# noirmist/Pytorch_Pose_Proposal_Network

Hardware: AMD Instinct MI355X
Metric: images/sec (384x384, DRN-D-22) at 1/2/4/8 MI355X (higher is better)
Workload: dtype bf16

## Files before the change

include/ppn.h:

```cpp
#ifndef PPN_H
#define PPN_H

#include <stddef.h>
#include <stdint.h>

#ifdef __cplusplus
extern "C" {
#endif

#define PPN_OK 0
#define PPN_E_INVALID (-1)
#define PPN_E_HIP (-2)
#define PPN_E_UNSUPPORTED (-3)

#define PPN_MAX_EDGES 32
#define PPN_MAX_KP 32

const char* ppn_last_error(void);
int ppn_version(void);

typedef struct ppn_decode_cfg {
    int32_t K, E;
    int32_t sH, sW;
    int32_t H, W;
// ... 113 lines not shown
#define PPN_CONV_NO_FILTER_BANK 1
#define PPN_CONV_SHARED_GPU 2
#define PPN_CONV_OUT_BF16 4
#define PPN_CONV_X3_PLAIN_OUT 8

int ppn_conv_tiling(int32_t dtype, int32_t cin, int32_t cout, int32_t ksize, int32_t* k_step, int32_t* cout_tile,
                    int32_t* k_order);

int ppn_conv2d_fused(const ppn_conv_desc* d, void* stream);

typedef struct ppn_block_desc {
    int32_t dtype;
    int32_t batch, h, w, channels;
    const void* src;
    const void* residual;
    const void* weight1;
    const float* scale_mid;
    const float* shift_mid;
    int32_t act_mid;
    const void* weight2;
    const float* scale1;
    const float* shift1;
    int32_t act1;
    const float* scale2;
    const float* shift2;
    int32_t act2;
    void* out_raw;
    void* out_act;
    int32_t flags;
    int32_t stride, in_h, in_w;
    const void* proj_src;
    const void* proj_weight;
    const float* proj_scale;
    const float* proj_shift;
    int32_t w1_ld, proj_ld;
} ppn_block_desc;
int ppn_basicblock64_fused(const ppn_block_desc* d, void* stream);

int ppn_pack_weight_x3(const float* w, int32_t cout, int32_t cin, int32_t ksize, int32_t cout_pad, int32_t scale_log2,
                       void* out, void* stream);
int ppn_split_f16x3(const float* src, int64_t pixels, int32_t channels, void* dst, void* stream);

int ppn_conv_split(int32_t dtype, int32_t cin, int32_t cout, int64_t m, int64_t* m_split);

int ppn_ingest_frames(const void* src_bgr, int32_t batch, int32_t src_h, int32_t src_w, void* dst_rgb, int32_t dst_h,
                      int32_t dst_w, int32_t flip, int32_t swap_rb, void* stream);

int ppn_set_conv_tile_policy(int32_t policy);

int ppn_set_conv_tile_override(int32_t bp, int32_t bc);

int ppn_set_conv64_enabled(int32_t on);

const char* ppn_last_conv_kernel(void);

int ppn_stem7x7(int32_t dtype, int32_t src_is_u8, const void* src, int32_t batch, int32_t h, int32_t w,
                const float* weight, const float* scale, const float* shift, const float* mean, const float* std_,
                void* out, void* stream);

int ppn_stem01(int32_t dtype, int32_t src_is_u8, const void* src, int32_t batch, int32_t h, int32_t w,
               const float* w0, const float* scale0, const float* shift0, const float* mean, const float* std_,
               const float* w1, const float* scale1, const float* shift1, void* out, void* stream);

typedef struct ppn_plan ppn_plan;
int ppn_plan_create(ppn_plan** out);
int ppn_plan_add_conv(ppn_plan* p, const ppn_conv_desc* d);
int ppn_plan_add_block(ppn_plan* p, const ppn_block_desc* d);
int ppn_plan_add_memset(ppn_plan* p, void* ptr, size_t bytes);
int ppn_plan_add_split(ppn_plan* p, const float* src, int64_t pixels, int32_t channels, void* dst);
int ppn_plan_add_stem(ppn_plan* p, int32_t dtype, int32_t src_is_u8, const void* src, int32_t batch, int32_t h,
                      int32_t w, const float* weight, const float* scale, const float* shift, const float* mean,
                      const float* std_, void* out);
int ppn_plan_add_stem01(ppn_plan* p, int32_t dtype, int32_t src_is_u8, const void* src, int32_t batch, int32_t h,
                        int32_t w, const float* w0, const float* scale0, const float* shift0, const float* mean,
                        const float* std_, const float* w1, const float* scale1, const float* shift1, void* out);
int ppn_stem012(int32_t src_is_u8, const void* src, int32_t batch, int32_t h, int32_t w, const float* w0,
                const float* scale0, const float* shift0, const float* mean, const float* std_, const float* w1,
                const float* scale1, const float* shift1, const float* w2, const float* scale2, const float* shift2,
                const float* scale3, const float* shift3, void* out_raw, void* out_act, void* stream);
int ppn_plan_add_stem012(ppn_plan* p, int32_t src_is_u8, const void* src, int32_t batch, int32_t h, int32_t w,
                         const float* w0, const float* scale0, const float* shift0, const float* mean, const float* std_,
                         const float* w1, const float* scale1, const float* shift1, const float* w2, const float* scale2,
                         const float* shift2, const float* scale3, const float* shift3, void* out_raw, void* out_act);
#define PPN_STEM_IO(internal, out) ((internal) | (((out) + 1) << 8))
#define PPN_STEM_RAW_S2 (1 << 16)
int ppn_stem012_dt(int32_t dtype, int32_t src_is_u8, const void* src, int32_t batch, int32_t h, int32_t w, const float* w0,
                   const float* scale0, const float* shift0, const float* mean, const float* std_, const float* w1,
                   const float* scale1, const float* shift1, const float* w2, const float* scale2, const float* shift2,
                   const float* scale3, const float* shift3, void* out_raw, void* out_act, void* stream);
int ppn_plan_add_stem012_dt(ppn_plan* p, int32_t dtype, int32_t src_is_u8, const void* src, int32_t batch, int32_t h,
                            int32_t w, const float* w0, const float* scale0, const float* shift0, const float* mean,
                            const float* std_, const float* w1, const float* scale1, const float* shift1, const float* w2,
                            const float* scale2, const float* shift2, const float* scale3, const float* shift3,
                            void* out_raw, void* out_act);
int ppn_plan_set_input(ppn_plan* p, const void* src);
int ppn_plan_run(ppn_plan* p, void* stream);
int ppn_plan_run_timed(ppn_plan* p, void* stream, float* ms, int32_t n_ms, int32_t repeats);
int ppn_plan_graph_captures(const ppn_plan* p);
int ppn_plan_size(const ppn_plan* p);
const char* ppn_plan_kernel_name(const ppn_plan* p, int32_t i);
int ppn_plan_destroy(ppn_plan* p);

int ppn_pack_weight(int32_t dtype, const float* w, int32_t cout, int32_t cin, int32_t ksize, int32_t cout_pad,
                    int32_t k_total, int32_t k_order, int32_t k_step, void* out, void* stream);
int ppn_pack_weight_dgrad(int32_t dtype, const float* w, int32_t cout, int32_t cin, int32_t ksize, int32_t cout_pad,
                          int32_t k_total, int32_t k_order, int32_t k_step, void* out, void* stream);
// ... 142 lines not shown
```

pytorch_pose_proposal_network_amd/csrc/conv_big.hip:

```cpp
#include <algorithm>
#include <cstdio>
#include <cstdlib>
#include <type_traits>
#include <utility>

#include "conv_common.h"

namespace {

using namespace ppnconv;

constexpr bool stats_tile_ok(int bp, int bc) {
    return bc >= 128 && (size_t)bp * (size_t)(bc * 2 + 16) <= 2 * (size_t)(bp + bc) * 128;
}

#ifndef PPN_DIAG
#define PPN_DIAG 0
#endif
constexpr unsigned kOOB = 0x80000000u;

template <typename F, int... I>
__device__ __forceinline__ void static_for_impl(F&& f, std::integer_sequence<int, I...>) {
    (f(std::integral_constant<int, I>{}), ...);
}
template <int N, typename F>
__device__ __forceinline__ void static_for(F&& f) {
    static_for_impl(f, std::make_integer_sequence<int, N>{});
}

template <typename T>
__device__ __forceinline__ void load4(const char* p, float* v);
template <>
__device__ __forceinline__ void load4<float>(const char* p, float* v) {
    const float4 a = *reinterpret_cast<const float4*>(p);
    v[0] = a.x; v[1] = a.y; v[2] = a.z; v[3] = a.w;
}
template <>
__device__ __forceinline__ void load4<__bf16>(const char* p, float* v) {
    const uint2 a = *reinterpret_cast<const uint2*>(p);
    v[0] = __uint_as_float(a.x << 16); v[1] = __uint_as_float(a.x & 0xffff0000u);
    v[2] = __uint_as_float(a.y << 16); v[3] = __uint_as_float(a.y & 0xffff0000u);
}
template <>
__device__ __forceinline__ void load4<_Float16>(const char* p, float* v) {
    typedef __attribute__((ext_vector_type(4))) _Float16 f16x4;
    const f16x4 a = *reinterpret_cast<const f16x4*>(p);
#pragma unroll
    for (int i = 0; i < 4; ++i) v[i] = (float)a[i];
}
template <typename T>
__device__ __forceinline__ void store4(char* p, const float* v);
template <>
__device__ __forceinline__ void store4<float>(char* p, const float* v) {
    *reinterpret_cast<float4*>(p) = make_float4(v[0], v[1], v[2], v[3]);
}
template <>
__device__ __forceinline__ void store4<__bf16>(char* p, const float* v) {
    typedef __attribute__((ext_vector_type(4))) __bf16 bf16x4;
    bf16x4 o;
#pragma unroll
    for (int i = 0; i < 4; ++i) o[i] = (__bf16)v[i];
    *reinterpret_cast<bf16x4*>(p) = o;
}

template <>
__device__ __forceinline__ void store4<_Float16>(char* p, const float* v) {
    typedef __attribute__((ext_vector_type(4))) _Float16 f16x4;
    f16x4 o;
#pragma unroll
    for (int i = 0; i < 4; ++i) o[i] = (_Float16)clamp_f16(v[i]);
    *reinterpret_cast<f16x4*>(p) = o;
}

__device__ __forceinline__ void bufload_lds16(__amdgpu_buffer_rsrc_t rsrc, char* lds_wave_base, unsigned voff,
                                              unsigned soff) {
    __builtin_amdgcn_raw_ptr_buffer_load_lds(rsrc, (void __attribute__((address_space(3)))*)lds_wave_base, 16, voff,
                                             soff, 0, 0);
}

template <typename T, int BP, int BC, int NW, bool SC, bool X3 = false, bool ST = false>
__global__ void __launch_bounds__(64 * NW, (ST && BP == 192 && BC == 128) ? 4 : NW / 4)
conv_igemm_big_kernel(ConvKArgs a, unsigned src_bytes, unsigned wgt_bytes) {
    static_assert(!X3 || (std::is_same<T, _Float16>::value && !SC), "X3 is the split-f16 mode without a fused shortcut");
    static_assert(!ST || (sizeof(T) == 2 && !SC && !X3 && NW == 8 && BC >= 128), "ST: plain 16-bit launches of the 8-wave tiles");
    constexpr int EPC = Elem<T>::EPC;
    constexpr int BK = 8 * EPC;
    constexpr int ES = sizeof(T);
    constexpr int NT = 64 * NW;
    constexpr int WC = (BP % (16 * (NW / 2)) == 0) ? 2 : NW;
    constexpr int WP = NW / WC;
    constexpr int NXI = (BP + 8 * NW - 1) / (8 * NW), NWI = BC / (8 * NW);
    constexpr bool XRAGGED = BP % (8 * NW) != 0;
    constexpr int TP = BP / WP / 16, TC = BC / WC / 16;
    constexpr int STAGE = (BP + BC) * 128;
    static_assert(BP % 8 == 0 && BC % (8 * NW) == 0 && (BP / WP) % 16 == 0 && BC % (16 * WC) == 0, "tile shape");
    static_assert(TP <= 9 && TC <= 8 && TC * TP % 2 == 0, "accumulators must fit the register file");

    extern __shared__ __attribute__((aligned(16))) char smem[];
#ifdef PPN_CLOCK
    const unsigned long long ck_entry = __builtin_amdgcn_s_memtime();
    const unsigned long long rk_entry = __builtin_amdgcn_s_memrealtime();
#endif
    const int tid = threadIdx.x, lane = tid & 63;
    const int wave = __builtin_amdgcn_readfirstlane(tid >> 6);
    const int wc = wave / WP, wp = wave % WP;

    int ptile, ctile;
    {
        const int nb = gridDim.x, id = blockIdx.x;
        const int xcd = id & 7, loc = id >> 3, q = nb >> 3, r = nb & 7;
        const int logical = (xcd < r ? xcd * (q + 1) : r * (q + 1) + (xcd - r) * q) + loc;
        ptile = fast_div(logical, a.div_nct);
        ctile = logical - ptile * a.n_ctiles;
    }
    const int m0 = a.m_base + ptile * BP, c0 = ctile * BC;

    const __amdgpu_buffer_rsrc_t xrs = __builtin_amdgcn_make_buffer_rsrc((void*)a.src, 0, src_bytes, 0x00020000);
    const __amdgpu_buffer_rsrc_t wrs = __builtin_amdgcn_make_buffer_rsrc((void*)a.wgt, 0, wgt_bytes, 0x00020000);
    const __amdgpu_buffer_rsrc_t xrs2 =
        __builtin_amdgcn_make_buffer_rsrc((void*)(SC ? a.src2 : a.src), 0, SC ? a.src2_bytes : 0u, 0x00020000);

    const int lrow = lane >> 3;
    const int chunk = (lane & 7) ^ (((lane >> 4) & 3) | ((wave & 1) << 2));
    const int ntaps = a.ks * a.ks;
    int xbase[NXI];
    int xbase2[NXI];
    unsigned xmask[NXI];
#pragma unroll
    for (int j = 0; j < NXI; ++j) {
        const int row = (j * NW + wave) * 8 + lrow;
        const int m = m0 + row;
        const bool vm = m < a.M;
        const int mm = vm ? m : 0;
        const int b = fast_div(mm, a.div_howo), rem = mm - b * a.HoWo;
        const int oy = fast_div(rem, a.div_wo), ox = rem - oy * a.Wo;
        const int iy0 = oy * a.stride - a.pad, ix0 = ox * a.stride - a.pad;
        xbase[j] = (((b * a.H + iy0) * a.W + ix0) * a.Cin + chunk * EPC) * ES;
        unsigned mk = 0, cx = 0;
#pragma unroll
        for (int dx = 0; dx < 5; ++dx)
            cx |= (dx < a.ks && (unsigned)(ix0 + dx * a.dil) < (unsigned)a.W) ? (1u << dx) : 0u;
#pragma unroll
        for (int dy = 0; dy < 5; ++dy)
            mk |= (dy < a.ks && (unsigned)(iy0 + dy * a.dil) < (unsigned)a.H) ? (cx << (dy * a.ks)) : 0u;
        mk = vm ? mk : 0u;
        xmask[j] = mk | (vm ? 0x80000000u : 0u);
        if constexpr (SC)
            xbase2[j] = (((b * a.H2 + oy * a.stride2) * a.W2 + ox * a.stride2) * a.Cin2 + chunk * EPC) * ES;
        else
            xbase2[j] = 0;
    }
    unsigned woff[NWI];
#pragma unroll
    for (int j = 0; j < NWI; ++j) {
        const int row = (j * NW + wave) * 8 + lrow;
        woff[j] = (unsigned)(((size_t)(c0 + row) * a.Ktot + chunk * EPC) * ES);
    }

    const int nsteps = a.Ktot / BK;
    const int dx_bytes = a.dil * a.Cin * ES;
    const int dy_bytes = a.dil * a.W * a.Cin * ES - a.ks * dx_bytes;
    const int ksz = a.ks;
    int u_tap = 0, u_dx = 0, u_slab = 0, tapoff = 0, u_ph = 0;
    unsigned tapbit = 1u;
    unsigned ksoff = 0;
    bool live = true;
    bool phase2 = a.nsteps_main == 0;
    int ld_step = 0;
// ... 74 lines not shown
            wf[r - TP] = *reinterpret_cast<const f32x4*>(smem + buf * STAGE + w_tile_off + foff[ks] + (r - TP) * 16 * 128);
    };
    constexpr int GS = (TC * TP % 4 == 0) ? 4 : ((TC * TP % 3 == 0) ? 3 : 2);
    constexpr int NG = TC * TP / GS;
#if PPN_DIAG == 3 || PPN_DIAG == 4
    typedef float f32x16 __attribute__((ext_vector_type(16)));
    f32x16 acc32[TC * TP / 4];
#pragma unroll
    for (int i = 0; i < TC * TP / 4; ++i)
#pragma unroll
        for (int j = 0; j < 16; ++j) acc32[i][j] = 0.f;
#endif
    auto mma_group = [&](auto gc, const f32x4 (&wf)[TC], const f32x4 (&xf)[TP]) {
        constexpr int g = decltype(gc)::value;
#if PPN_DIAG == 3 || PPN_DIAG == 4
        if constexpr (std::is_same<T, __bf16>::value) {
            constexpr int i0 = g * 4, i1 = g * 4 + 3;
            acc32[g] = __builtin_amdgcn_mfma_f32_32x32x16_bf16(__builtin_bit_cast(bf16x8, wf[i0 / TP]),
                                                               __builtin_bit_cast(bf16x8, xf[i0 % TP]), acc32[g], 0, 0, 0);
            acc32[g] = __builtin_amdgcn_mfma_f32_32x32x16_bf16(__builtin_bit_cast(bf16x8, wf[i1 / TP]),
                                                               __builtin_bit_cast(bf16x8, xf[i1 % TP]), acc32[g], 0, 0, 0);
            return;
        }
#endif
        static_for<GS>([&](auto tc) {
            constexpr int idx = g * GS + decltype(tc)::value;
            mma_step(acc[idx / TP][idx % TP], wf[idx / TP], xf[idx % TP], (T*)nullptr);
        });
    };
    constexpr int RPG = (NRD + NG - 1) / NG;
    constexpr int LPG = (NL + NG - 1) / NG;

#ifdef PPN_CLOCK
    const unsigned long long ck_state = __builtin_amdgcn_s_memtime();
#endif
    static_for<NL>([&](auto gc) { issue_one(gc, 0); });
    advance();
    static_for<NL>([&](auto gc) { issue_one(gc, 1); });
    advance();
    if constexpr (XRAGGED) {
        if ((NXI - 1) * NW * 8 + wave * 8 < BP) asm volatile("s_waitcnt vmcnt(%0)" ::"n"(NL) : "memory");
        else asm volatile("s_waitcnt vmcnt(%0)" ::"n"(NL - 1) : "memory");
    } else {
        asm volatile("s_waitcnt vmcnt(%0)" ::"n"(NL) : "memory");
    }
    __syncthreads();
#ifdef PPN_CLOCK
    const unsigned long long ck_bar = __builtin_amdgcn_s_memtime();
#endif
    static_for<NRD>([&](auto rc) { read_one(rc, wA, xA, 0, 0); });
    static_for<NRD>([&](auto rc) { read_one(rc, wB, xB, 0, 1); });
    static_for<NG>([&](auto gc) { mma_group(gc, wA, xA); });
    asm volatile("s_waitcnt vmcnt(0) lgkmcnt(0)" ::: "memory");
    __syncthreads();

#ifdef PPN_STAMP
    unsigned long long st_b1 = 0, st_b2 = 0, st_wait = 0, st_bar = 0, tq0, tq1;
#define PPN_T(var) do { __builtin_amdgcn_sched_barrier(0); asm volatile("s_memtime %0\n\ts_waitcnt lgkmcnt(0)" : "=s"(var) :: "memory"); __builtin_amdgcn_sched_barrier(0); } while (0)
#else
#define PPN_T(var) do { } while (0)
#endif
#ifdef PPN_CLOCK
    const unsigned long long ck0 = __builtin_amdgcn_s_memtime(), rk0 = __builtin_amdgcn_s_memrealtime();
#endif
    for (int s = 1; s < nsteps; ++s) {
        const int buf = s & 1;
#ifdef PPN_STAMP
        PPN_T(tq0);
#endif
        static_for<NG>([&](auto gc) {
            constexpr int g = decltype(gc)::value;
            mma_group(gc, wB, xB);
#if PPN_DIAG != 2 && PPN_DIAG != 4 && PPN_DIAG != 5 && PPN_DIAG != 6
            static_for<LPG>([&](auto lc) {
                constexpr int l = g * LPG + decltype(lc)::value;
                if constexpr (l < NL) issue_one(std::integral_constant<int, l>{}, buf ^ 1);
            });
#endif
            static_for<RPG>([&](auto rc) {
                constexpr int r = g * RPG + decltype(rc)::value;
                if constexpr (r < NRD) read_one(std::integral_constant<int, r>{}, wA, xA, buf, 0);
            });
            __builtin_amdgcn_sched_barrier(0);
        });
        advance();
#ifdef PPN_STAMP
        PPN_T(tq1); st_b1 += tq1 - tq0;
#endif
        static_for<NG>([&](auto gc) {
            constexpr int g = decltype(gc)::value;
            mma_group(gc, wA, xA);
            static_for<RPG>([&](auto rc) {
                constexpr int r = g * RPG + decltype(rc)::value;
                if constexpr (r < NRD) read_one(std::integral_constant<int, r>{}, wB, xB, buf, 1);
            });
            __builtin_amdgcn_sched_barrier(0);
        });
#ifdef PPN_STAMP
        PPN_T(tq0); st_b2 += tq0 - tq1;
#endif
#if PPN_DIAG == 1
        asm volatile("s_waitcnt lgkmcnt(0)" ::: "memory");
#else
        asm volatile("s_waitcnt vmcnt(0) lgkmcnt(0)" ::: "memory");
#endif
#ifdef PPN_STAMP
        PPN_T(tq1); st_wait += tq1 - tq0;
#endif
#if PPN_DIAG != 5
        __syncthreads();
#endif
#ifdef PPN_STAMP
        PPN_T(tq0); st_bar += tq0 - tq1;
#endif
    }
#ifdef PPN_CLOCK
    {
        const unsigned long long ck1 = __builtin_amdgcn_s_memtime(), rk1 = __builtin_amdgcn_s_memrealtime();
        if (lane == 0 && a.scale2 == nullptr && a.shift2 != nullptr) {
            unsigned long long* dbg = (unsigned long long*)a.shift2 + ((size_t)blockIdx.x * NW + wave) * 8;
            dbg[0] = ck1 - ck0; dbg[1] = rk1 - rk0; dbg[2] = ck0 - ck_entry; dbg[3] = ck1; dbg[5] = ck_state - ck_entry; dbg[6] = ck_bar - ck_entry;
        }
    }
#endif
#ifdef PPN_STAMP
    unsigned long long t_epi0;
    PPN_T(t_epi0);
    if (lane == 0 && a.scale2 == nullptr && a.shift2 != nullptr) {
        unsigned long long* dbg = (unsigned long long*)a.shift2 + ((size_t)blockIdx.x * NW + wave) * 8;
        dbg[0] = st_b1; dbg[1] = st_b2; dbg[2] = st_wait; dbg[3] = st_bar;
    }
#endif
    static_for<NG>([&](auto gc) { mma_group(gc, wB, xB); });
#if PPN_DIAG == 3 || PPN_DIAG == 4
#pragma unroll
    for (int i = 0; i < TC * TP / 4; ++i)
#pragma unroll
        for (int j = 0; j < 16; ++j) acc[(i * 4 + j / 4) / TP][(i * 4 + j / 4) % TP][j % 4] += acc32[i][j];
#endif
    __syncthreads();

    int pf_keep0 = 0, pf_keep1 = 0;
    if (a.pf_per_wg) {
        const unsigned l0 = blockIdx.x * a.pf_per_wg + tid, lend = min((blockIdx.x + 1) * a.pf_per_wg, a.pf_lines);
        if (l0 < lend) pf_keep0 = *reinterpret_cast<const int*>(a.pf_ptr + (size_t)l0 * 128);
        if (l0 + 64 * NW < lend) pf_keep1 = *reinterpret_cast<const int*>(a.pf_ptr + (size_t)(l0 + 64 * NW) * 128);
        asm volatile("" : "+v"(pf_keep0), "+v"(pf_keep1));
    }

    float* ct = reinterpret_cast<float*>(smem);
    constexpr int RS16 = BC * 2 + 16;
#ifdef PPN_NO_FAST_EPI
    constexpr bool kFastFits = false;
#else
    constexpr bool kFastFits = !X3 && sizeof(T) == 2 && BC >= 128 && (size_t)BP * RS16 <= 2 * (size_t)STAGE;
#endif
#ifndef PPN_NO_FAST_EPI
    static_assert(!ST || kFastFits, "ST lives in the single-output 16-bit epilogue");
#endif
    bool fast = false;
    if constexpr (kFastFits) fast = !a.nchw && !a.residual && !a.out_act && a.out_raw && (a.Cout & 7) == 0 && !a.out_bf16;
    if (fast) {
        if constexpr (kFastFits) {
            const float slope1 = a.act1 == PPN_ACT_RELU ? 0.f : (a.act1 == PPN_ACT_LRELU ? 0.1f : 1.f);
            const bool al = (!a.scale1 || (reinterpret_cast<size_t>(a.scale1) & 15) == 0) &&
                            (!a.shift1 || (reinterpret_cast<size_t>(a.shift1) & 15) == 0);
#pragma unroll
            for (int i = 0; i < TC; ++i) {
                const int chl = wc * (BC / WC) + i * 16 + 4 * fq;
                const int c = c0 + chl;
                float sc[4] = {1.f, 1.f, 1.f, 1.f}, sh[4] = {0.f, 0.f, 0.f, 0.f};
                if (al && c + 4 <= a.Cout) {
                    if (a.scale1) { const float4 t = *reinterpret_cast<const float4*>(a.scale1 + c); sc[0] = t.x; sc[1] = t.y; sc[2] = t.z; sc[3] = t.w; }
                    if (a.shift1) { const float4 t = *reinterpret_cast<const float4*>(a.shift1 + c); sh[0] = t.x; sh[1] = t.y; sh[2] = t.z; sh[3] = t.w; }
                } else {
#pragma unroll
                    for (int r = 0; r < 4; ++r) {
                        if (a.scale1 && c + r < a.Cout) sc[r] = a.scale1[c + r];
                        if (a.shift1 && c + r < a.Cout) sh[r] = a.shift1[c + r];
                    }
                }
#pragma unroll
                for (int j = 0; j < TP; ++j) {
                    const int px = wp * (BP / WP) + j * 16 + frow;
                    float v[4];
#pragma unroll
                    for (int r = 0; r < 4; ++r) {
                        const float t1 = acc[i][j][r] * sc[r] + sh[r];
                        v[r] = fmaxf(t1, t1 * slope1);
                    }
                    store4<T>(smem + px * RS16 + chl * 2, v);
                }
            }
            constexpr int CPR = BC / 8;
            constexpr int NQ = BP * CPR / NT;
            static_assert(BP * CPR % NT == 0, "tile must split into whole 16-byte chunks per thread");
            const size_t row_bytes = (size_t)a.Cout * 2;
            static_assert(!ST || NT % CPR == 0, "ST: a thread keeps its chunk column");
            uint4 sx[ST ? NQ : 1];
            float st_sc[8], st_sh[8], st_mu[8], st_rs[8], st_s0[8], st_s1[8];
            float st_neg = 1.f;
            const int st_mode = ST ? a.st_mode : 0;
            if constexpr (ST) {
#pragma unroll
                for (int j = 0; j < 8; ++j) st_s0[j] = st_s1[j] = 0.f;
                if (st_mode == 2) {
                    const int cc = tid % CPR, c = c0 + cc * 8;
                    const bool vc = c < a.Cout;
                    static_for<NQ>([&](auto qc) {
                        constexpr int q = decltype(qc)::value;
                        const int m = m0 + q * (NT / CPR) + tid / CPR;
                        sx[q] = (vc && m < a.M) ? *reinterpret_cast<const uint4*>(a.st_x + (size_t)m * row_bytes + (size_t)c * 2)
                                                : make_uint4(0u, 0u, 0u, 0u);
                    });
// ... 46 lines not shown
                                const float xh = (x[j] - st_mu[j]) * st_rs[j];
                                st_s0[j] += g;
                                st_s1[j] = fmaf(g, xh, st_s1[j]);
                            }
                        }
                    }
                }
            };
            if constexpr (!ST) {
#pragma unroll
                for (int q = 0; q < NQ; ++q) {
                    const int id = q * NT + tid;
                    const int px = id / CPR, cc = id % CPR;
                    const int m = m0 + px, c = c0 + cc * 8;
                    if (m < a.M && c < a.Cout) {
                        const uint4 o = *reinterpret_cast<const uint4*>(smem + px * RS16 + cc * 16);
                        *reinterpret_cast<uint4*>(a.out_raw + (size_t)m * row_bytes + (size_t)c * 2) = o;
                    }
                }
            } else {
                if (st_mode == 0) static_for<NQ>([&](auto qc) { store_chunk(qc, std::integral_constant<int, 0>{}); });
                if (st_mode == 1) static_for<NQ>([&](auto qc) { store_chunk(qc, std::integral_constant<int, 1>{}); });
                if (st_mode == 2) static_for<NQ>([&](auto qc) { store_chunk(qc, std::integral_constant<int, 2>{}); });
            }
            if constexpr (ST) {
                if (st_mode != 0) {
#pragma unroll
                    for (int off = 32; off >= CPR; off >>= 1)
#pragma unroll
                        for (int j = 0; j < 8; ++j) {
                            st_s0[j] += __shfl_xor(st_s0[j], off, 64);
                            st_s1[j] += __shfl_xor(st_s1[j], off, 64);
                        }
                    lds_barrier();
                    float* red = reinterpret_cast<float*>(smem);
                    if (lane < CPR) {
#pragma unroll
                        for (int j = 0; j < 8; ++j) {
                            red[(wave * CPR + lane) * 16 + j] = st_s0[j];
                            red[(wave * CPR + lane) * 16 + 8 + j] = st_s1[j];
                        }
                    }
                    lds_barrier();
                    if (tid < CPR * 16) {
                        const int ccx = tid >> 4, j = tid & 15;
                        double acc = 0.0;
#pragma unroll
                        for (int w = 0; w < NW; ++w) acc += (double)red[(w * CPR + ccx) * 16 + j];
                        const int ch = c0 + ccx * 8 + (j & 7);
                        if (ch < a.Cout) a.st_partial[((size_t)ptile * a.Cout + ch) * 2 + (j >> 3)] = acc;
                    }
                }
            }
        }
    } else if (!a.nchw) {
        constexpr int LD = BC + 4;
        constexpr int JC = (TP % 2 == 0 && WP == 2) ? 2 : 1;
        constexpr int CPX = WP * JC * 16;
        constexpr int TPP = BC / 8, PPP = NT / TPP;
        static_assert(TP % JC == 0 && CPX % PPP == 0, "epilogue chunking");
        static_assert((size_t)CPX * LD * 4 <= 2 * (size_t)STAGE, "epilogue chunk must fit the staging LDS");
        const int cg = tid % TPP, prow = tid / TPP;
        const int c = c0 + cg * 8;
        const float slope1 = a.act1 == PPN_ACT_RELU ? 0.f : (a.act1 == PPN_ACT_LRELU ? 0.1f : 1.f);
        const float slope2 = a.act2 == PPN_ACT_RELU ? 0.f : (a.act2 == PPN_ACT_LRELU ? 0.1f : 1.f);
        float s1[8], b1[8], s2[8], b2[8];
        auto affine8 = [&](const float* p, float dflt, float* o) {
            if (p && c + 8 <= a.Cout && (reinterpret_cast<size_t>(p) & 15) == 0) {
                const float4 lo = *reinterpret_cast<const float4*>(p + c), hi = *reinterpret_cast<const float4*>(p + c + 4);
                o[0] = lo.x; o[1] = lo.y; o[2] = lo.z; o[3] = lo.w; o[4] = hi.x; o[5] = hi.y; o[6] = hi.z; o[7] = hi.w;
            } else {
#pragma unroll
                for (int i = 0; i < 8; ++i) o[i] = (p && c + i < a.Cout) ? p[c + i] : dflt;
            }
        };
        affine8(a.scale1, 1.f, s1); affine8(a.shift1, 0.f, b1);
        affine8(a.scale2, 1.f, s2); affine8(a.shift2, 0.f, b2);
#ifdef PPN_CLOCK
        unsigned long long ep_w = 0, ep_s = 0;
#endif
        auto chunk = [&](auto qc) {
            constexpr int q = decltype(qc)::value;
#ifdef PPN_CLOCK
            const unsigned long long e0 = __builtin_amdgcn_s_memtime();
#endif
#pragma unroll
            for (int jj = 0; jj < JC; ++jj)
#pragma unroll
                for (int i = 0; i < TC; ++i) {
                    const int px = (wp * JC + jj) * 16 + frow;
                    const int ch = wc * (BC / WC) + i * 16 + 4 * fq;
                    *reinterpret_cast<f32x4*>(ct + px * LD + ch) = acc[i][q * JC + jj];
                }
            lds_barrier();
#ifdef PPN_CLOCK
            const unsigned long long e1 = __builtin_amdgcn_s_memtime();
#endif
            if (c < a.Cout) {
                constexpr int NPASS = CPX / PPP;
                int mrow[NPASS];
                size_t moff[NPASS];
                float res[NPASS][8];
                const size_t row_bytes = (size_t)a.Cout * ES * (X3 ? 2 : 1);
                const size_t lo_bytes = (size_t)a.Cout * ES;
#pragma unroll
                for (int pass = 0; pass < NPASS; ++pass) {
// ... 170 lines not shown
            for (int item = tid; item < NITEM; item += NT) {
                const int chl = item / TPC, pq = item - chl * TPC;
                const int cw = chl / (IC * 16), ci = (chl / 16) % IC, cr = chl % 16;
                const int c = c0 + cw * (BC / WC) + (q * IC + ci) * 16 + cr;
                const int m = m0 + 4 * pq;
                if (c < a.Cout && m < a.M) {
                    const f32x4 t4 = *reinterpret_cast<const f32x4*>(ct + chl * LD + 4 * pq);
                    float v[4] = {t4.x, t4.y, t4.z, t4.w};
#pragma unroll
                    for (int i = 0; i < 4; ++i) v[i] = apply_act(v[i], a.act1);
                    if (vec) {
                        const int nb = fast_div(m, a.div_howo), np = m - nb * a.HoWo;
                        *reinterpret_cast<float4*>(out + ((size_t)nb * a.Cout + c) * a.HoWo + np) =
                            make_float4(v[0], v[1], v[2], v[3]);
                    } else {
#pragma unroll
                        for (int i = 0; i < 4; ++i) {
                            const int mi = m + i;
                            if (mi < a.M) {
                                const int bi = fast_div(mi, a.div_howo), pi = mi - bi * a.HoWo;
                                out[((size_t)bi * a.Cout + c) * a.HoWo + pi] = v[i];
                            }
                        }
                    }
                }
            }
            lds_barrier();
        };
        static_for<TC / IC>(chunk);
    }
    asm volatile("" ::"v"(pf_keep0), "v"(pf_keep1));
#ifdef PPN_CLOCK
    if (lane == 0 && a.scale2 == nullptr && a.shift2 != nullptr) {
        unsigned long long* dbg = (unsigned long long*)a.shift2 + ((size_t)blockIdx.x * NW + wave) * 8;
        dbg[4] = __builtin_amdgcn_s_memtime() - dbg[3];
#if PPN_CLOCK + 0 >= 2
        dbg[5] = rk_entry; dbg[6] = __builtin_amdgcn_s_memrealtime();
#endif
    }
    (void)rk_entry;
#endif
#ifdef PPN_STAMP
    {
        unsigned long long t_epi1;
        PPN_T(t_epi1);
        if (lane == 0 && a.scale2 == nullptr && a.shift2 != nullptr) {
            unsigned long long* dbg = (unsigned long long*)a.shift2 + ((size_t)blockIdx.x * NW + wave) * 8;
            dbg[4] = t_epi1 - t_epi0;
        }
    }
#endif
}

template <typename T, int BP, int BC, int NW, bool SC, bool X3 = false, bool ST = false>
int launch_sc(const ConvKArgs& a, hipStream_t st, const char** kname) {
    constexpr size_t lds = 2 * (size_t)(BP + BC) * 128;
    static char name[96];
    if (!name[0])
        snprintf(name, sizeof(name), "conv_igemm_big_kernel<%s, %d, %d, %d, %s%s>", elem_name<T>(),
                 BP, BC, NW, SC ? "true" : "false", X3 ? ", true" : (ST ? ", false, true" : ""));
    if (kname) *kname = name;
    const size_t src_bytes = (size_t)a.B * a.H * a.W * a.Cin * sizeof(T);
    const size_t wgt_bytes = (size_t)a.n_ctiles * BC * a.Ktot * sizeof(T);
    auto k = conv_igemm_big_kernel<T, BP, BC, NW, SC, X3, ST>;
    {
        static int max_lds_set = 0;
        PPN_LDS_ONCE(max_lds_set, reinterpret_cast<const void*>(k), hipFuncAttributeMaxDynamicSharedMemorySize,
                                      (int)lds);
    }
    ConvKArgs b = a;
    if (b.pf_lines) {
        const unsigned nwg = (unsigned)(a.n_ctiles * a.n_ptiles);
        b.pf_per_wg = std::min<unsigned>((b.pf_lines + nwg - 1) / nwg, 2u * 64 * NW);
    }
    hipLaunchKernelGGL(k, dim3(a.n_ctiles * a.n_ptiles), dim3(64 * NW), lds, st, b, (unsigned)src_bytes,
                       (unsigned)wgt_bytes);
    PPN_LAUNCH_CHECK();
    return PPN_OK;
}

template <typename T, int BP, int BC, int NW>
int launch_one(const ConvKArgs& a, hipStream_t st, const char** kname) {
    if constexpr (NW == 8 && BC >= 128) {
        if (a.src2) return launch_sc<T, BP, BC, NW, true>(a, st, kname);
    } else {
        if (a.src2) return ppn::fail(PPN_E_UNSUPPORTED, "fused shortcut needs the 8-wave 128/256-channel tiles");
    }
    if (a.st_mode != 0) {
        if constexpr (std::is_same<T, __bf16>::value && NW == 8 && stats_tile_ok(BP, BC))
            return launch_sc<T, BP, BC, NW, false, false, true>(a, st, kname);
        else
            return ppn::fail(PPN_E_UNSUPPORTED, "BatchNorm statistics: no such instantiation of the large-tile kernel");
    }
    return launch_sc<T, BP, BC, NW, false>(a, st, kname);
}

int conv_waves() {
    static const int nw = getenv("PPN_CONV_WAVES") ? atoi(getenv("PPN_CONV_WAVES")) : 8;
    return nw;
}

template <typename T>
int launch_T(const ConvKArgs& a, BigTile t, hipStream_t st, const char** kname) {
    const int nw = conv_waves();
    if (nw == 4 && t.bp != 144) {
        if (t.bc == 256) {
            if (t.bp == 256) return launch_one<T, 256, 256, 4>(a, st, kname);
            if (t.bp == 192) return launch_one<T, 192, 256, 4>(a, st, kname);
            return launch_one<T, 128, 256, 4>(a, st, kname);
        }
        if (t.bp == 256) return launch_one<T, 256, 128, 4>(a, st, kname);
        if (t.bp == 192) return launch_one<T, 192, 128, 4>(a, st, kname);
        return launch_one<T, 128, 128, 4>(a, st, kname);
    }
    if (t.bc == 256) {
        if (t.bp == 256) return launch_one<T, 256, 256, 8>(a, st, kname);
        if (t.bp == 192) return launch_one<T, 192, 256, 8>(a, st, kname);
        if (t.bp == 144) return launch_one<T, 144, 256, 8>(a, st, kname);
        return launch_one<T, 128, 256, 8>(a, st, kname);
    }
    if (t.bc == 128) {
        if (t.bp == 256) return launch_one<T, 256, 128, 8>(a, st, kname);
        if (t.bp == 192) return launch_one<T, 192, 128, 8>(a, st, kname);
// ... 73 lines not shown
long long big_split_for(int cout, long long m) {
    BigTile single;
    if (g_tile_policy != 2 || cout < 256 || cout >= 4096 || !big_tile_for(cout, m, &single) || g_ov_bp > 0) return 0;
    struct Cand { int bp, bc; double eff; };
    static const Cand cands[] = {{256, 256, 1.27}, {192, 256, 1.10}, {128, 256, 0.92}, {256, 128, 0.90},
                                 {192, 128, 0.95}, {128, 128, 0.87}};
    auto rounds_cost = [&](const Cand& cd, long long mm) {
        const long long tiles = ((mm + cd.bp - 1) / cd.bp) * ((cout + cd.bc - 1) / cd.bc);
        return (double)((tiles + 255) / 256) * cd.bp * cd.bc / cd.eff;
    };
    double best_single = 1e30;
    for (const Cand& cd : cands) best_single = std::min(best_single, rounds_cost(cd, m));
    double best = best_single * 0.96;
    long long cut = 0;
    for (const Cand& p : cands) {
        const long long ct = (cout + p.bc - 1) / p.bc;
        if (256 % ct != 0) continue;
        const long long rounds = (m / p.bp) * ct / 256;
        if (rounds < 1) continue;
        const long long m1 = rounds * 256 / ct * p.bp;
        if (m1 >= m) continue;
        double tail = 1e30;
        for (const Cand& q : cands) tail = std::min(tail, rounds_cost(q, m - m1));
        const double cost = (double)rounds * p.bp * p.bc / p.eff + tail;
        if (cost < best) { best = cost; cut = m1; }
    }
    return cut;
}

bool big_stats_ok(int dtype, BigTile t) {
    return dtype == PPN_BF16 && conv_waves() == 8 && stats_tile_ok(t.bp, t.bc);
}

int launch_big(const ConvKArgs& a, int dtype, BigTile t, hipStream_t st, const char** kname) {
    const size_t es = dtype == PPN_F32 ? 4 : 2;
    if ((size_t)a.B * a.H * a.W * a.Cin * es >= 0x7fffff00ull || (size_t)a.n_ctiles * t.bc * a.Ktot * es >= 0x7fffff00ull)
        return ppn::fail(PPN_E_UNSUPPORTED, "tensor too large for the buffer-addressed conv kernel");
    if (dtype == PPN_F32) return launch_T<float>(a, t, st, kname);
    if (dtype == PPN_F16X3) return launch_X3(a, t, st, kname);
    if (dtype == PPN_F16) return launch_T<_Float16>(a, t, st, kname);
    return launch_T<__bf16>(a, t, st, kname);
}

}

extern "C" int ppn_set_conv_tile_override(int32_t bp, int32_t bc) {
    if (bp == 0 && bc == 0) { ppnconv::g_ov_bp = ppnconv::g_ov_bc = 0; return PPN_OK; }
    if (!ppnconv::tile_shape_ok(bp, bc))
        return ppn::fail(PPN_E_INVALID, "ppn_set_conv_tile_override: bp in {128,192,256}, bc in {64,128,256}, not 192x64; or 144x256");
    ppnconv::g_ov_bp = bp; ppnconv::g_ov_bc = bc;
    return PPN_OK;
}

extern "C" int ppn_set_conv_tile_policy(int32_t policy) {
    if (policy < 0 || policy > 2) return ppn::fail(PPN_E_INVALID, "ppn_set_conv_tile_policy: 0, 1 or 2");
    ppnconv::g_tile_policy = policy;
    return PPN_OK;
}
```

pytorch_pose_proposal_network_amd/csrc/conv_common.h:

```cpp
#pragma once
#include <hip/hip_bf16.h>

#include "common.h"

namespace ppnconv {

typedef __attribute__((ext_vector_type(4))) float f32x4;
typedef __attribute__((ext_vector_type(8))) short s16x8;
typedef __attribute__((ext_vector_type(8))) __bf16 bf16x8;
typedef __attribute__((ext_vector_type(8))) _Float16 f16x8;

struct FastDiv {
    unsigned mul, sh1, sh2;
};
inline FastDiv make_fastdiv(unsigned d) {
    unsigned l = 0;
    while ((1ull << l) < d) ++l;
    const unsigned long long m = ((1ull << 32) * ((1ull << l) - d)) / d + 1;
    return FastDiv{(unsigned)m, l < 1 ? l : 1u, l > 0 ? l - 1 : 0u};
}
__device__ __forceinline__ int fast_div(int n, const FastDiv& f) {
    const unsigned t = __umulhi(f.mul, (unsigned)n);
    return (int)((t + (((unsigned)n - t) >> f.sh1)) >> f.sh2);
}

struct ConvKArgs {
    const char* src;
    const char* wgt;
    const float* scale1;
    const float* shift1;
    const char* residual;
    char* out_raw;
    const float* scale2;
    const float* shift2;
    char* out_act;
    const char* zero;
    int B, H, W, Cin, Ho, Wo, Cout, ks, stride, dil, pad;
    int Ktot;
    int M;
    int m_base;
    int HoWo;
    FastDiv div_howo, div_wo, div_nct;
    int act1, act2, nchw;
    int log2Cin;
    int n_ctiles, n_ptiles;
    float* unary_out;
    unsigned long long* amax_keys;
    int unary_ch, window;
    const char* src2;
    int H2, W2, Cin2, stride2;
    int nsteps_main;
    unsigned src2_bytes;
    int lo_off;
    int out_bf16;
    int out_plain;
    const char* pf_ptr;
    unsigned pf_lines, pf_per_wg;
    double* st_partial;
    int st_mode, st_act;
    const char* st_x;
    const float *st_gamma, *st_beta, *st_mean, *st_rstd;
};

template <typename T>
struct Elem;
template <>
struct Elem<float> {
    static constexpr int EPC = 4;
};
template <>
struct Elem<__bf16> {
    static constexpr int EPC = 8;
};
template <>
struct Elem<_Float16> {
    static constexpr int EPC = 8;
};
template <typename T> constexpr const char* elem_name() { return sizeof(T) == 4 ? "float" : "__bf16"; }
template <> constexpr const char* elem_name<_Float16>() { return "_Float16"; }

__device__ __forceinline__ float sigmoid_fast(float v) { return __builtin_amdgcn_rcpf(1.0f + __expf(-v)); }

__device__ __forceinline__ float apply_act(float v, int act) {
    switch (act) {
        case PPN_ACT_RELU: return v > 0.f ? v : 0.f;
        case PPN_ACT_LRELU: return v > 0.f ? v : v * 0.1f;
        case PPN_ACT_SIGMOID: return sigmoid_fast(v);
        default: return v;
    }
}

__device__ __forceinline__ void glds16(const char* gptr, char* lds_wave_base) {
    __builtin_amdgcn_global_load_lds((const void __attribute__((address_space(1)))*)gptr,
                                     (void __attribute__((address_space(3)))*)lds_wave_base, 16, 0, 0);
}

__device__ __forceinline__ void mma_step(f32x4& acc, const f32x4& wf, const f32x4& xf, float*) {
    acc = __builtin_amdgcn_mfma_f32_16x16x4f32(wf.x, xf.x, acc, 0, 0, 0);
    acc = __builtin_amdgcn_mfma_f32_16x16x4f32(wf.y, xf.y, acc, 0, 0, 0);
    acc = __builtin_amdgcn_mfma_f32_16x16x4f32(wf.z, xf.z, acc, 0, 0, 0);
    acc = __builtin_amdgcn_mfma_f32_16x16x4f32(wf.w, xf.w, acc, 0, 0, 0);
}
__device__ __forceinline__ void mma_step(f32x4& acc, const f32x4& wf, const f32x4& xf, __bf16*) {
    acc = __builtin_amdgcn_mfma_f32_16x16x32_bf16(__builtin_bit_cast(bf16x8, wf), __builtin_bit_cast(bf16x8, xf),
                                                  acc, 0, 0, 0);
}

__device__ __forceinline__ void mma_step(f32x4& acc, const f32x4& wf, const f32x4& xf, _Float16*) {
    acc = __builtin_amdgcn_mfma_f32_16x16x32_f16(__builtin_bit_cast(f16x8, wf), __builtin_bit_cast(f16x8, xf), acc, 0, 0, 0);
}

template <typename T>
__device__ __forceinline__ void load8(const char* p, float* v);
template <>
// ... 73 lines not shown
```

pytorch_pose_proposal_network_amd/lib.py:

```python
from __future__ import annotations

import ctypes as C
import os

_HERE = os.path.dirname(os.path.abspath(__file__))
LIB_PATH = os.environ.get("PPN_LIB", os.path.join(_HERE, "csrc", "libppn.so"))

PPN_MAX_EDGES = 32
PPN_MAX_KP = 32
PPN_F32, PPN_BF16, PPN_F16, PPN_F16X3 = 0, 1, 2, 3
PPN_CONV_NO_FILTER_BANK, PPN_CONV_SHARED_GPU, PPN_CONV_OUT_BF16, PPN_CONV_X3_PLAIN_OUT = 1, 2, 4, 8
PPN_ACT_NONE, PPN_ACT_RELU, PPN_ACT_LRELU, PPN_ACT_SIGMOID = 0, 1, 2, 3
PPN_STEM_RAW_S2 = 1 << 16


def PPN_STEM_IO(internal: int, out: int) -> int:
    return internal | ((out + 1) << 8)


PPN_STEM_X3_F32 = PPN_STEM_IO(PPN_F16X3, PPN_F32)


class DecodeCfg(C.Structure):
    _fields_ = [
# ... 61 lines not shown


class BnBwdDesc(C.Structure):
    _fields_ = [("dtype", C.c_int32), ("channels", C.c_int32), ("pixels", C.c_int64), ("act", C.c_int32)] + [
        (n, C.c_void_p) for n in ("x", "dy", "dx_add", "gamma", "beta", "save_mean", "save_rstd", "dgamma", "dbeta",
                                  "dx", "workspace")] + [("stats_blocks", C.c_int32)] + [
        (n, C.c_void_p) for n in ("next_x", "next_gamma", "next_beta", "next_mean", "next_rstd")] + [
        ("next_act", C.c_int32), ("next_blocks", C.POINTER(C.c_int32))]


class WgradDesc(C.Structure):
    _fields_ = [(n, C.c_int32) for n in ("dtype", "batch", "in_h", "in_w", "cin", "out_h", "out_w", "cout", "ksize",
                                         "stride", "dilation", "pad")] + [
        ("beta", C.c_float), ("x", C.c_void_p), ("dy", C.c_void_p), ("dw", C.c_void_p), ("workspace", C.c_void_p),
        ("workspace_bytes", C.c_uint64)]


class PPNError(RuntimeError):
    pass


_lib = None

_SIGNATURES = {
    "ppn_last_error": (C.c_char_p, []),
    "ppn_version": (C.c_int, []),
    "ppn_decode_workspace_bytes": (C.c_size_t, [C.POINTER(DecodeCfg), C.c_int32]),
    "ppn_decode": (C.c_int, [C.POINTER(DecodeCfg), C.c_void_p, C.c_int32, C.c_void_p, C.c_void_p, C.c_void_p,
                             C.c_void_p, C.c_void_p, C.c_void_p, C.c_void_p]),
    "ppn_decode_fused": (C.c_int, [C.POINTER(DecodeCfg), C.c_void_p, C.c_void_p, C.c_int32, C.c_void_p, C.c_void_p,
                                   C.c_void_p, C.c_void_p, C.c_void_p, C.c_void_p]),
    "ppn_decode_fused_workspace_bytes": (C.c_size_t, [C.POINTER(DecodeCfg), C.c_int32]),
    "ppn_decode_fused_ws": (C.c_int, [C.POINTER(DecodeCfg), C.c_void_p, C.c_void_p, C.c_int32, C.c_void_p, C.c_void_p,
                                      C.c_void_p, C.c_void_p, C.c_void_p, C.c_void_p, C.c_void_p]),
    "ppn_limb_argmax": (C.c_int, [C.POINTER(DecodeCfg), C.c_void_p, C.c_int32, C.c_void_p, C.c_void_p]),
    "ppn_nms": (C.c_int, [C.c_void_p, C.c_void_p, C.c_int32, C.c_float, C.c_int32, C.c_void_p, C.c_void_p,
                          C.c_void_p]),
    "ppn_loss_workspace_bytes": (C.c_size_t, [C.POINTER(LossCfg), C.c_int32]),
    "ppn_loss_fwd_bwd": (C.c_int, [C.POINTER(LossCfg), C.c_void_p, C.c_int32] + [C.c_void_p] * 10 +
                         [C.POINTER(C.c_float), C.c_void_p, C.c_void_p, C.c_void_p, C.c_void_p]),
    "ppn_loss_dz_workspace_bytes": (C.c_size_t, [C.POINTER(LossCfg), C.c_int32, C.c_int32]),
    "ppn_loss_fwd_bwd_dz": (C.c_int, [C.POINTER(LossCfg), C.c_void_p, C.c_int32] + [C.c_void_p] * 10 +
                            [C.c_void_p, C.c_float, C.c_void_p, C.c_void_p, C.c_int32, C.c_int32, C.c_void_p, C.c_void_p,
                             C.c_void_p, C.c_void_p]),
    "ppn_loss_fwd_bwd_dz_c": (C.c_int, [C.POINTER(LossCfg), C.c_void_p, C.c_int32] + [C.c_void_p] * 9 +
                              [C.c_void_p, C.c_float, C.c_void_p, C.c_void_p, C.c_int32, C.c_int32, C.c_void_p, C.c_void_p,
                               C.c_void_p, C.c_void_p]),
    "ppn_loss_fwd_bwd_dev": (C.c_int, [C.POINTER(LossCfg), C.c_void_p, C.c_int32] + [C.c_void_p] * 10 +
                             [C.c_void_p, C.c_float, C.c_void_p, C.c_void_p, C.c_void_p, C.c_void_p]),
    "ppn_conv_tiling": (C.c_int, [C.c_int32, C.c_int32, C.c_int32, C.c_int32, C.POINTER(C.c_int32),
                                  C.POINTER(C.c_int32), C.POINTER(C.c_int32)]),
    "ppn_conv2d_fused": (C.c_int, [C.POINTER(ConvDesc), C.c_void_p]),
    "ppn_set_conv64_enabled": (C.c_int, [C.c_int32]),
    "ppn_basicblock64_fused": (C.c_int, [C.POINTER(BlockDesc), C.c_void_p]),
    "ppn_conv_split": (C.c_int, [C.c_int32, C.c_int32, C.c_int32, C.c_int64, C.POINTER(C.c_int64)]),
    "ppn_stem7x7": (C.c_int, [C.c_int32, C.c_int32, C.c_void_p, C.c_int32, C.c_int32, C.c_int32] +
                    [C.c_void_p] * 3 + [C.POINTER(C.c_float)] * 2 + [C.c_void_p, C.c_void_p]),
    "ppn_stem01": (C.c_int, [C.c_int32, C.c_int32, C.c_void_p, C.c_int32, C.c_int32, C.c_int32] + [C.c_void_p] * 3 +
                   [C.POINTER(C.c_float)] * 2 + [C.c_void_p] * 5),
    "ppn_plan_add_stem01": (C.c_int, [C.c_void_p, C.c_int32, C.c_int32, C.c_void_p, C.c_int32, C.c_int32, C.c_int32] +
                            [C.c_void_p] * 3 + [C.POINTER(C.c_float)] * 2 + [C.c_void_p] * 4),
    "ppn_stem012": (C.c_int, [C.c_int32, C.c_void_p, C.c_int32, C.c_int32, C.c_int32] + [C.c_void_p] * 3 +
                    [C.POINTER(C.c_float)] * 2 + [C.c_void_p] * 11),
    "ppn_plan_add_stem012": (C.c_int, [C.c_void_p, C.c_int32, C.c_void_p, C.c_int32, C.c_int32, C.c_int32] +
                             [C.c_void_p] * 3 + [C.POINTER(C.c_float)] * 2 + [C.c_void_p] * 10),
    "ppn_stem012_dt": (C.c_int, [C.c_int32, C.c_int32, C.c_void_p, C.c_int32, C.c_int32, C.c_int32] + [C.c_void_p] * 3 +
                       [C.POINTER(C.c_float)] * 2 + [C.c_void_p] * 11),
    "ppn_plan_add_stem012_dt": (C.c_int, [C.c_void_p, C.c_int32, C.c_int32, C.c_void_p, C.c_int32, C.c_int32, C.c_int32] +
                                [C.c_void_p] * 3 + [C.POINTER(C.c_float)] * 2 + [C.c_void_p] * 10),
    "ppn_plan_create": (C.c_int, [C.POINTER(C.c_void_p)]),
    "ppn_plan_add_conv": (C.c_int, [C.c_void_p, C.POINTER(ConvDesc)]),
    "ppn_plan_add_block": (C.c_int, [C.c_void_p, C.POINTER(BlockDesc)]),
    "ppn_plan_add_memset": (C.c_int, [C.c_void_p, C.c_void_p, C.c_size_t]),
    "ppn_plan_add_split": (C.c_int, [C.c_void_p, C.c_void_p, C.c_int64, C.c_int32, C.c_void_p]),
    "ppn_pack_weight_x3": (C.c_int, [C.c_void_p, C.c_int32, C.c_int32, C.c_int32, C.c_int32, C.c_int32, C.c_void_p,
                                     C.c_void_p]),
    "ppn_split_f16x3": (C.c_int, [C.c_void_p, C.c_int64, C.c_int32, C.c_void_p, C.c_void_p]),
    "ppn_plan_add_stem": (C.c_int, [C.c_void_p, C.c_int32, C.c_int32, C.c_void_p, C.c_int32, C.c_int32, C.c_int32] +
                          [C.c_void_p] * 3 + [C.POINTER(C.c_float)] * 2 + [C.c_void_p]),
    "ppn_plan_set_input": (C.c_int, [C.c_void_p, C.c_void_p]),
    "ppn_plan_run": (C.c_int, [C.c_void_p, C.c_void_p]),
    "ppn_plan_run_timed": (C.c_int, [C.c_void_p, C.c_void_p, C.POINTER(C.c_float), C.c_int32, C.c_int32]),
    "ppn_plan_size": (C.c_int, [C.c_void_p]),
    "ppn_plan_graph_captures": (C.c_int, [C.c_void_p]),
    "ppn_plan_kernel_name": (C.c_char_p, [C.c_void_p, C.c_int32]),
    "ppn_plan_destroy": (C.c_int, [C.c_void_p]),
    "ppn_pack_weight": (C.c_int, [C.c_int32, C.c_void_p, C.c_int32, C.c_int32, C.c_int32, C.c_int32, C.c_int32,
                                  C.c_int32, C.c_int32, C.c_void_p, C.c_void_p]),
    "ppn_pack_weight_dgrad": (C.c_int, [C.c_int32, C.c_void_p, C.c_int32, C.c_int32, C.c_int32, C.c_int32, C.c_int32,
                                  C.c_int32, C.c_int32, C.c_void_p, C.c_void_p]),
    "ppn_pack_table_build": (C.c_int, [C.POINTER(PackItem), C.c_int32, C.c_void_p, C.POINTER(C.c_int32)]),
    "ppn_pack_table_run": (C.c_int, [C.c_void_p, C.c_int32, C.c_int32, C.c_void_p]),
}

_SIGNATURES.update({
    "ppn_bn_workspace_bytes": (C.c_size_t, [C.c_int32]),
    "ppn_bn_train_fwd": (C.c_int, [C.POINTER(BnDesc), C.c_void_p]),
    "ppn_bn_train_bwd": (C.c_int, [C.POINTER(BnBwdDesc), C.c_void_p]),
    "ppn_adam_step": (C.c_int, [C.c_void_p, C.c_void_p, C.c_void_p, C.c_void_p, C.c_int64, C.c_double, C.c_double,
                                C.c_double, C.c_double, C.c_double, C.c_int32, C.c_float, C.c_void_p, C.c_void_p]),
    "ppn_sumsq": (C.c_int, [C.c_void_p, C.c_int64, C.c_void_p, C.c_void_p, C.c_void_p]),
    "ppn_gradnorm_probe_stats": (C.c_int, [C.c_void_p] * 5 + [C.POINTER(C.c_float), C.c_int64, C.c_void_p, C.c_void_p,
                                           C.c_void_p, C.c_void_p]),
    "ppn_gradnorm_weight_step": (C.c_int, [C.c_void_p, C.c_void_p, C.c_void_p, C.c_void_p, C.c_float, C.c_void_p,
                                           C.c_void_p, C.c_double, C.c_double, C.c_double, C.c_double, C.c_int32,
                                           C.c_void_p, C.c_void_p]),
# ... 88 lines not shown
```

Before: 11430.

## Add one-pass residual epilogue and early residual prefetch in big conv kernel

Adds a new non-fast epilogue path that loads the residual tile into registers directly from global memory, applies affine, activation and residual add, stages the result through LDS, and writes it with 16-byte coalesced stores, optionally followed by a second affine/activation output. It also touches the residual rows before the main loop so they are warm in cache by epilogue time (mode 1 by default, or mid-loop in mode 2). Both are gated by a runtime epilogue mode flag that defaults to on. The aim is to cut epilogue latency and the cost of the generic multi-pass store path, at the cost of extra registers, more LDS barriers and extra memory traffic from the prefetch.

New measurement: 11140. -2.5%, worse.

```diff
diff --git a/include/ppn.h b/include/ppn.h
--- a/include/ppn.h
+++ b/include/ppn.h
@@ -189,6 +189,8 @@
 
 int ppn_set_conv64_enabled(int32_t on);
 
+int ppn_set_conv_epilogue_mode(int32_t mode);
+
 const char* ppn_last_conv_kernel(void);
 
 int ppn_stem7x7(int32_t dtype, int32_t src_is_u8, const void* src, int32_t batch, int32_t h, int32_t w,
diff --git a/pytorch_pose_proposal_network_amd/csrc/conv_big.hip b/pytorch_pose_proposal_network_amd/csrc/conv_big.hip
--- a/pytorch_pose_proposal_network_amd/csrc/conv_big.hip
+++ b/pytorch_pose_proposal_network_amd/csrc/conv_big.hip
@@ -16,6 +16,12 @@
 
 #ifndef PPN_DIAG
 #define PPN_DIAG 0
+#endif
+#ifndef PPN_RES_PF
+#define PPN_RES_PF 1
+#endif
+#ifndef PPN_RES_PF_STEPS
+#define PPN_RES_PF_STEPS 4
 #endif
 constexpr unsigned kOOB = 0x80000000u;
 
@@ -114,6 +120,30 @@
         ctile = logical - ptile * a.n_ctiles;
     }
     const int m0 = a.m_base + ptile * BP, c0 = ctile * BC;
+
+    constexpr bool kResPf = PPN_RES_PF != 0 && sizeof(T) == 2 && !X3 && !ST;
+    constexpr int RLR = BC / 64;
+    constexpr int NRL = (BP * RLR + 64 * NW - 1) / (64 * NW);
+    int rpf[NRL];
+#pragma unroll
+    for (int k = 0; k < NRL; ++k) rpf[k] = 0;
+    auto touch_residual = [&]() {
+#pragma unroll
+        for (int k = 0; k < NRL; ++k) {
+            const int l = k * (64 * NW) + (int)threadIdx.x;
+            const int row = l / RLR, c = c0 + (l % RLR) * 64;
+            if (row < BP && m0 + row < a.M && c < a.Cout && (a.Cout & 1) == 0)
+                rpf[k] = *reinterpret_cast<const int*>(a.residual + ((size_t)(m0 + row) * a.Cout + c) * 2);
+        }
+#pragma unroll
+        for (int k = 0; k < NRL; ++k) asm volatile("" : "+v"(rpf[k]));
+    };
+    auto sink_residual = [&]() {
+#pragma unroll
+        for (int k = 0; k < NRL; ++k) asm volatile("" ::"v"(rpf[k]));
+    };
+    if constexpr (kResPf && PPN_RES_PF == 1)
+        if (a.residual && (a.epi_mode & 2)) touch_residual();
 
     const __amdgpu_buffer_rsrc_t xrs = __builtin_amdgcn_make_buffer_rsrc((void*)a.src, 0, src_bytes, 0x00020000);
     const __amdgpu_buffer_rsrc_t wrs = __builtin_amdgcn_make_buffer_rsrc((void*)a.wgt, 0, wgt_bytes, 0x00020000);
@@ -294,6 +324,7 @@
     static_for<NRD>([&](auto rc) { read_one(rc, wB, xB, 0, 1); });
     static_for<NG>([&](auto gc) { mma_group(gc, wA, xA); });
     asm volatile("s_waitcnt vmcnt(0) lgkmcnt(0)" ::: "memory");
+    if constexpr (kResPf && PPN_RES_PF == 1) sink_residual();
     __syncthreads();
 
 #ifdef PPN_STAMP
@@ -305,7 +336,7 @@
 #ifdef PPN_CLOCK
     const unsigned long long ck0 = __builtin_amdgcn_s_memtime(), rk0 = __builtin_amdgcn_s_memrealtime();
 #endif
-    for (int s = 1; s < nsteps; ++s) {
+    auto kstep = [&](int s) {
         const int buf = s & 1;
 #ifdef PPN_STAMP
         PPN_T(tq0);
@@ -355,6 +386,15 @@
 #ifdef PPN_STAMP
         PPN_T(tq0); st_bar += tq0 - tq1;
 #endif
+    };
+    if constexpr (kResPf && PPN_RES_PF == 2) {
+        const bool pf = a.residual && (a.epi_mode & 2);
+        const int nsplit = pf ? max(nsteps - PPN_RES_PF_STEPS, 1) : nsteps;
+        for (int s = 1; s < nsplit; ++s) kstep(s);
+        if (pf) touch_residual();
+        for (int s = nsplit; s < nsteps; ++s) kstep(s);
+    } else {
+        for (int s = 1; s < nsteps; ++s) kstep(s);
     }
 #ifdef PPN_CLOCK
     {
@@ -380,6 +420,7 @@
 #pragma unroll
         for (int j = 0; j < 16; ++j) acc[(i * 4 + j / 4) / TP][(i * 4 + j / 4) % TP][j % 4] += acc32[i][j];
 #endif
+    if constexpr (kResPf && PPN_RES_PF == 2) sink_residual();
     __syncthreads();
 
     int pf_keep0 = 0, pf_keep1 = 0;
@@ -402,6 +443,9 @@
 #endif
     bool fast = false;
     if constexpr (kFastFits) fast = !a.nchw && !a.residual && !a.out_act && a.out_raw && (a.Cout & 7) == 0 && !a.out_bf16;
+    constexpr bool kOnePass = kFastFits && !ST && !(NW == 8 && BP == 128 && BC == 256);
+    bool onepass = false;
+    if constexpr (kOnePass) onepass = !fast && !a.nchw && (a.Cout & 7) == 0 && !a.out_bf16 && (a.epi_mode & 1);
     if (fast) {
         if constexpr (kFastFits) {
             const float slope1 = a.act1 == PPN_ACT_RELU ? 0.f : (a.act1 == PPN_ACT_LRELU ? 0.1f : 1.f);
@@ -554,6 +598,108 @@
                     }
                 }
             }
+        }
+    } else if (onepass) {
+        if constexpr (kOnePass) {
+            const float slope1 = a.act1 == PPN_ACT_RELU ? 0.f : (a.act1 == PPN_ACT_LRELU ? 0.1f : 1.f);
+            const float slope2 = a.act2 == PPN_ACT_RELU ? 0.f : (a.act2 == PPN_ACT_LRELU ? 0.1f : 1.f);
+            const size_t row_bytes = (size_t)a.Cout * 2;
+#ifdef PPN_CLOCK
+            const unsigned long long e0 = __builtin_amdgcn_s_memtime();
+#endif
+            uint2 rs[TC][TP];
+#pragma unroll
+            for (int j = 0; j < TP; ++j) {
+                const int m = m0 + wp * (BP / WP) + j * 16 + frow;
+                const char* rrow = a.residual + (size_t)m * row_bytes;
+#pragma unroll
+                for (int i = 0; i < TC; ++i) {
+                    const int c = c0 + wc * (BC / WC) + i * 16 + 4 * fq;
+                    rs[i][j] = (a.residual && m < a.M && c < a.Cout) ? *reinterpret_cast<const uint2*>(rrow + (size_t)c * 2)
+                                                                     : make_uint2(0u, 0u);
+                }
+            }
+            auto affine4 = [&](const float* p, int c, float dflt, float* o) {
+                if (p && c + 4 <= a.Cout && (reinterpret_cast<size_t>(p) & 15) == 0) {
+                    const float4 t = *reinterpret_cast<const float4*>(p + c);
+                    o[0] = t.x; o[1] = t.y; o[2] = t.z; o[3] = t.w;
+                } else {
+#pragma unroll
+                    for (int r = 0; r < 4; ++r) o[r] = (p && c + r < a.Cout) ? p[c + r] : dflt;
+                }
+            };
+            constexpr int CPR = BC / 8;
+            constexpr int NQ = BP * CPR / NT;
+            static_assert(BP * CPR % NT == 0, "tile must split into whole 16-byte chunks per thread");
+            auto flush16 = [&](char* dst) {
+#pragma unroll
+                for (int q = 0; q < NQ; ++q) {
+                    const int id = q * NT + tid;
+                    const int px = id / CPR, cc = id % CPR;
+                    const int m = m0 + px, c = c0 + cc * 8;
+                    if (m < a.M && c < a.Cout) {
+                        const uint4 o = *reinterpret_cast<const uint4*>(smem + px * RS16 + cc * 16);
+                        *reinterpret_cast<uint4*>(dst + (size_t)m * row_bytes + (size_t)c * 2) = o;
+                    }
+                }
+            };
+#pragma unroll
+            for (int i = 0; i < TC; ++i) {
+                const int chl = wc * (BC / WC) + i * 16 + 4 * fq;
+                float sc[4], sh[4];
+                affine4(a.scale1, c0 + chl, 1.f, sc); affine4(a.shift1, c0 + chl, 0.f, sh);
+#pragma unroll
+                for (int j = 0; j < TP; ++j) {
+                    const int px = wp * (BP / WP) + j * 16 + frow;
+                    float res[4], v[4];
+                    load4<T>(reinterpret_cast<const char*>(&rs[i][j]), res);
+#pragma unroll
+                    for (int r = 0; r < 4; ++r) {
+                        const float t1 = acc[i][j][r] * sc[r] + sh[r];
+                        v[r] = fmaxf(t1, t1 * slope1) + res[r];
+                        acc[i][j][r] = v[r];
+                    }
+                    if (a.out_raw) store4<T>(smem + px * RS16 + chl * 2, v);
+                }
+            }
+#ifdef PPN_CLOCK
+            unsigned long long e1 = __builtin_amdgcn_s_memtime();
+#endif
+            if (a.out_raw) {
+                lds_barrier();
+#ifdef PPN_CLOCK
+                e1 = __builtin_amdgcn_s_memtime();
+#endif
+                flush16(a.out_raw);
+                if (a.out_act) lds_barrier();
+            }
+            if (a.out_act) {
+#pragma unroll
+                for (int i = 0; i < TC; ++i) {
+                    const int chl = wc * (BC / WC) + i * 16 + 4 * fq;
+                    float sc[4], sh[4];
+                    affine4(a.scale2, c0 + chl, 1.f, sc); affine4(a.shift2, c0 + chl, 0.f, sh);
+#pragma unroll
+                    for (int j = 0; j < TP; ++j) {
+                        const int px = wp * (BP / WP) + j * 16 + frow;
+                        float u[4];
+#pragma unroll
+                        for (int r = 0; r < 4; ++r) {
+                            const float t2 = acc[i][j][r] * sc[r] + sh[r];
+                            u[r] = fmaxf(t2, t2 * slope2);
+                        }
+                        store4<T>(smem + px * RS16 + chl * 2, u);
+                    }
+                }
+                lds_barrier();
+                flush16(a.out_act);
+            }
+#ifdef PPN_CLOCK
+            if (lane == 0 && a.scale2 == nullptr && a.shift2 != nullptr) {
+                unsigned long long* dbg = (unsigned long long*)a.shift2 + ((size_t)blockIdx.x * NW + wave) * 8;
+                dbg[7] = ((e1 - e0) << 32) | (__builtin_amdgcn_s_memtime() - e1);
+            }
+#endif
         }
     } else if (!a.nchw) {
         constexpr int LD = BC + 4;
@@ -830,6 +976,8 @@
 #endif
 }
 
+int g_epi_mode = getenv("PPN_CONV_EPI") ? atoi(getenv("PPN_CONV_EPI")) & 3 : 3;
+
 template <typename T, int BP, int BC, int NW, bool SC, bool X3 = false, bool ST = false>
 int launch_sc(const ConvKArgs& a, hipStream_t st, const char** kname) {
     constexpr size_t lds = 2 * (size_t)(BP + BC) * 128;
@@ -847,6 +995,7 @@
                                       (int)lds);
     }
     ConvKArgs b = a;
+    b.epi_mode = g_epi_mode;
     if (b.pf_lines) {
         const unsigned nwg = (unsigned)(a.n_ctiles * a.n_ptiles);
         b.pf_per_wg = std::min<unsigned>((b.pf_lines + nwg - 1) / nwg, 2u * 64 * NW);
@@ -1026,6 +1175,12 @@
     return PPN_OK;
 }
 
+extern "C" int ppn_set_conv_epilogue_mode(int32_t mode) {
+    if (mode < 0 || mode > 3) return ppn::fail(PPN_E_INVALID, "ppn_set_conv_epilogue_mode: 0 .. 3");
+    g_epi_mode = mode;
+    return PPN_OK;
+}
+
 extern "C" int ppn_set_conv_tile_policy(int32_t policy) {
     if (policy < 0 || policy > 2) return ppn::fail(PPN_E_INVALID, "ppn_set_conv_tile_policy: 0, 1 or 2");
     ppnconv::g_tile_policy = policy;
diff --git a/pytorch_pose_proposal_network_amd/csrc/conv_common.h b/pytorch_pose_proposal_network_amd/csrc/conv_common.h
--- a/pytorch_pose_proposal_network_amd/csrc/conv_common.h
+++ b/pytorch_pose_proposal_network_amd/csrc/conv_common.h
@@ -60,6 +60,7 @@
     int st_mode, st_act;
     const char* st_x;
     const float *st_gamma, *st_beta, *st_mean, *st_rstd;
+    int epi_mode;
 };
 
 template <typename T>
diff --git a/pytorch_pose_proposal_network_amd/lib.py b/pytorch_pose_proposal_network_amd/lib.py
--- a/pytorch_pose_proposal_network_amd/lib.py
+++ b/pytorch_pose_proposal_network_amd/lib.py
@@ -137,6 +137,7 @@
                                   C.POINTER(C.c_int32), C.POINTER(C.c_int32)]),
     "ppn_conv2d_fused": (C.c_int, [C.POINTER(ConvDesc), C.c_void_p]),
     "ppn_set_conv64_enabled": (C.c_int, [C.c_int32]),
+    "ppn_set_conv_epilogue_mode": (C.c_int, [C.c_int32]),
     "ppn_basicblock64_fused": (C.c_int, [C.POINTER(BlockDesc), C.c_void_p]),
     "ppn_conv_split": (C.c_int, [C.c_int32, C.c_int32, C.c_int32, C.c_int64, C.POINTER(C.c_int64)]),
     "ppn_stem7x7": (C.c_int, [C.c_int32, C.c_int32, C.c_void_p, C.c_int32, C.c_int32, C.c_int32] +
```
